# wheaton5/cellector

Measured on AMD Instinct MI355X. Metric: cell x locus log-likelihood evals/sec over full EM iterations (EM iters/sec in em_iters_per_s), higher is better.
Workload: dtype f64

## Files before the change

### cellector_amd/csrc/kernels_tiled.hip

```cpp
#include <hip/hip_ext.h>

#include "tiled.h"

__device__ __constant__ uint8_t T_A_OF[T_NCODE] = {1, 0, 2, 1, 0, 3, 2, 1, 0, 4, 3, 2, 1, 0};
__device__ __constant__ uint8_t T_R_OF[T_NCODE] = {0, 1, 0, 1, 2, 0, 1, 2, 3, 0, 1, 2, 3, 4};

struct ab_src_t {
    const double *s_alt, *s_ref, *alt_min, *ref_min;
    const uint8_t *mask;
    double2 *ab_out;
    double *xl_counters;
    uint32_t *d_counters, *tile_work;
    uint32_t n_work;
};
template <bool PAIRS>
__global__ __launch_bounds__(64 * TB_PARTS) void k_build_tables(uint64_t L, uint32_t nj, const double2 *__restrict__ ab,
                                                                const double *__restrict__ lf, double *__restrict__ tab,
                                                                ab_src_t src)
{
    if (src.s_alt && blockIdx.x == 0) {
        if (threadIdx.x < LC_COUNTERS) src.xl_counters[threadIdx.x] = 0.0;
        if (threadIdx.x < 8) src.d_counters[threadIdx.x] = 0u;
        for (uint32_t i = threadIdx.x; i < src.n_work; i += blockDim.x) src.tile_work[i] = 0u;
    }
    const int part = threadIdx.x >> 6;
    const uint64_t t = (uint64_t)blockIdx.x * 64 + (threadIdx.x & 63);
    if (t >= (uint64_t)nj * T_BL) return;
    const uint64_t chunk = t / T_BL, slot = t % T_BL;
    const uint64_t l = chunk * T_BLU + slot;
    double2 p = make_double2(-1.0, -1.0);
    if (slot < T_BLU && l < L) {
        if (src.s_alt) {
            p.x = (src.s_alt[l] + 1.0) - src.alt_min[l];
            p.y = (src.s_ref[l] + 1.0) - src.ref_min[l];
            if (!src.mask[l]) p.x = p.y = -1.0;
            if (part == 0) src.ab_out[l] = p;
        } else {
            p = ab[l];
        }
    }
    const bool live = p.x >= 0.0;
    double *img = tab + chunk * TAB_ELEMS;
#define TB_PMF(W, A, R) img[tab_pmf<geo_reg>((uint32_t)slot, W)] = live ? dm_log_bb_pmf(lf, p.x, p.y, A, R) : 0.0
#define TB_EXP(N) img[tab_exp<geo_reg>((uint32_t)slot, N - 1)] = (PAIRS && live) ? dm_expected_log_pmf(lf, p.x, p.y, N) : 0.0
    switch (part) {
    case 0: TB_EXP(4u); TB_PMF(0, 1u, 0u); break;
    case 1: TB_EXP(3u); TB_PMF(1, 0u, 1u); break;
    case 2: TB_EXP(2u); TB_PMF(2, 2u, 0u); TB_PMF(3, 1u, 1u); break;
    case 3: TB_EXP(1u); TB_PMF(4, 0u, 2u); TB_PMF(5, 3u, 0u); break;
    case 4: TB_PMF(6, 2u, 1u); TB_PMF(7, 1u, 2u); TB_PMF(8, 0u, 3u); TB_PMF(9, 4u, 0u); break;
    default: TB_PMF(10, 3u, 1u); TB_PMF(11, 2u, 2u); TB_PMF(12, 1u, 3u); TB_PMF(13, 0u, 4u); break;
    }
#undef TB_PMF
#undef TB_EXP
}

#ifndef TILE_ABL
#define TILE_ABL 0
#endif
#ifndef TILE_PFD
#define TILE_PFD 2
#endif
#ifndef TILE_PFD_T2
#define TILE_PFD_T2 2
#endif
#ifndef TILE_PINNED
#define TILE_PINNED 1
#endif
#if TILE_ABL == 7
#define TILE_BARRIER() do { } while (0)
#else
#define TILE_BARRIER() asm volatile("s_waitcnt lgkmcnt(0)\n\ts_barrier" ::: "memory")
#endif

struct __attribute__((packed, aligned(4))) tile_u4 { uint32_t x, y, z, w; };

template <bool EXPECTED, int T_SB, class G = geo_reg>
__global__ __launch_bounds__(T_THREADS, 4) void k_tile_ll(uint32_t nb, uint32_t nj, uint32_t cpg, uint32_t groups,
                                                          uint32_t n_cols, uint32_t *__restrict__ work ,
                                                          const uint16_t *__restrict__ thdr,
                                                          const uint16_t *__restrict__ tiles,
                                                          const double *__restrict__ tab, uint64_t npad,
                                                          double *__restrict__ part_ll, double *__restrict__ part_ell)
{
    using tab_t = typename std::conditional<EXPECTED, double2, double>::type;
    constexpr uint32_t TAB_U = G::LROW * G::BL * sizeof(double) / 16;
    constexpr int NP = (TAB_U + T_THREADS - 1) / T_THREADS;
    static_assert(NP == 6, "table prefetch registers are written out by hand");
    __shared__ __attribute__((aligned(16))) double s_tab[G::LROW * G::BL];
    static_assert(G::LROW * G::BL % 2 == 0, "whole 16-byte units");
    __shared__ tab_t s_acc[T_SB * T_BC];
    __shared__ uint32_t s_col;
    const uint32_t tid = threadIdx.x, wv = tid >> 6, lane = tid & 63;
    const uint32_t g = blockIdx.x % groups;
    const uint32_t j0 = g * cpg, j1 = min(nj, j0 + cpg);
    if (j0 >= j1) return;
  for (;;) {
    if (tid == 0) s_col = atomicAdd(&work[g], 1u);
    __syncthreads();
    const uint32_t col = s_col;
    if (col >= n_cols) break;
    const uint32_t b0 = col * T_SB;
#pragma unroll
    for (int s = 0; s < T_SB; s++) {
        if constexpr (EXPECTED) s_acc[s * T_BC + tid] = make_double2(0.0, 0.0);
        else s_acc[s * T_BC + tid] = 0.0;
    }

    double2 p_t0, p_t1, p_t2, p_t3, p_t4, p_t5;
#define TABLE_PREFETCH(J)                                                                                        \
    do {                                                                                                         \
        const double2 *src__ = reinterpret_cast<const double2 *>(tab) + (uint64_t)(J) * TAB_U + tid;             \
        p_t0 = src__[0];                                                                                         \
        p_t1 = src__[T_THREADS];                                                                                 \
        p_t2 = src__[2 * T_THREADS];                                                                             \
        p_t3 = src__[3 * T_THREADS];                                                                             \
        p_t4 = src__[4 * T_THREADS];                                                                             \
        p_t5 = src__[5 * T_THREADS];                      \
    } while (0)

    struct row_t { tile_u4 lo, hi; uint32_t k; uint64_t base; };
    const uint32_t wv_s = (uint32_t)__builtin_amdgcn_readfirstlane((int)wv);
#define HDR_LOAD(H, J, S)            \
    do {                                                                                                         \
         \
         \
         \
        const uint32_t rot__ = (wv_s + 8u * ((uint32_t)(S) >> 1)) & 15u, sl__ = ((S) & 1u) ? 15u - rot__ : rot__; \
        if (TILE_ABL != 9 || first_rows)  \
        (H) = reinterpret_cast<const uint4 *>(thdr + ((uint64_t)min(b0 + (uint32_t)(S), nb - 1) * nj + (TILE_ABL == 10 ? j0 : (J))) * T_HDR)[sl__]; \
    } while (0)
#define ROW_LOAD(E, H)                                                                                           \
    do {                                                                                                         \
        (E).k = (SKIP_EMPTY && (H).w) ? 0u : (H).z;  \
        (E).base = ((uint64_t)(H).y << 32) | (H).x;                                                              \
         \
         \
        const char *sb__ = reinterpret_cast<const char *>(tiles + (E).base);                                     \
        const uint32_t off__ = __umul24(lane, ((H).z + 1u) * 2u);                      \
        if ((!(TILE_ABL == 2 || TILE_ABL == 9) || first_rows) && !(SKIP_EMPTY && (H).w)) {  \
            (E).lo = *reinterpret_cast<const tile_u4 *>(sb__ + off__);                                           \
            (E).hi = *reinterpret_cast<const tile_u4 *>(sb__ + ((H).z > 7u ? 16u : 0u) + off__);                 \
        }                                                                                                        \
    } while (0)

    constexpr bool SKIP_EMPTY = G::NLO != 1;
    constexpr uint32_t PFD = T_SB == 4 ? (uint32_t)(G::NLO == 1 ? TILE_PFD : TILE_PFD_T2) : 2u;
    static_assert(PFD >= 2 && PFD <= 4, "row buffers");
    uint4 h0, h1, h2, h3;
    row_t e0, e1, e2, e3;
    bool first_rows = true;
    TABLE_PREFETCH(j0);
    __builtin_amdgcn_sched_barrier(0);
#define HDR_STEP(H, T) HDR_LOAD(H, min(j0 + (uint32_t)(T) / T_SB, j1 - 1), (uint32_t)(T) % T_SB)
    HDR_STEP(h0, 0);
    HDR_STEP(h1, 1);
    if constexpr (PFD >= 3) HDR_STEP(h2, 2);
    if constexpr (PFD == 4) HDR_STEP(h3, 3);
    ROW_LOAD(e0, h0);
    ROW_LOAD(e1, h1);
    if constexpr (PFD >= 3) ROW_LOAD(e2, h2);
    if constexpr (PFD == 4) ROW_LOAD(e3, h3);
    HDR_STEP(h0, PFD);
    HDR_STEP(h1, PFD + 1);
    if constexpr (PFD >= 3) HDR_STEP(h2, PFD + 2);
    if constexpr (PFD == 4) HDR_STEP(h3, PFD + 3);
#undef HDR_STEP
    first_rows = false;

#if TILE_ABL == 1 || TILE_ABL == 5
#define TILE_LOOKUP(V, E16) do { if constexpr (EXPECTED) V = make_double2((double)(E16), 1.0); else V = (double)(E16); } while (0)
#elif TILE_ABL == 4
#define TILE_LOOKUP(V, E16)                                                                                      \
    do {                                                                                                         \
        const uint32_t b__ = (((E16) >> 4) & 127u) * 32u + (lane & 31u), c__ = (((E16) >> 5) & 127u) * 32u + (lane & 31u); \
        if constexpr (EXPECTED) V = make_double2(s_tab[b__], s_tab[c__ + 4096u]);                                \
        else V = s_tab[b__];                                                                                     \
    } while (0)
#else
#define TILE_LOOKUP(V, E16)                                                                                      \
    do {                                                                                                         \
        const uint32_t s__ = ((E16) >> G::SHIFT) & G::SMASK;                                                     \
        if constexpr (EXPECTED) V = make_double2(s_tab[tab_pmf<G>(s__, (E16) & G::CMASK)], s_tab[tab_exp<G>(s__, (E16) >> 14)]); \
        else V = s_tab[tab_pmf<G>(s__, (E16) & G::CMASK)];                                                       \
    } while (0)
#endif
#define TILE_RD(V, KK)                                                                                           \
    tab_t V;                                                                                                     \
    do {                                                                                                         \
        const uint32_t idx__ = (((KK) + 1) & 1) ? (w__[((KK) + 1) >> 1] >> 16) : (w__[((KK) + 1) >> 1] & 0xffffu); \
        TILE_LOOKUP(V, idx__);                                                                                   \
    } while (0)
#define TILE_ADD(V)                                                                                              \
    do {                                                                                                         \
        if constexpr (EXPECTED) { a_ll__ += (V).x; a_el__ += (V).y; }                                            \
        else a_ll__ += (V);                                                                                      \
    } while (0)
#if TILE_PINNED
#define TILE_PIN(V)                                                                                              \
    do {                                                                                                         \
        if constexpr (EXPECTED) asm volatile("" : "+v"((V).x), "+v"((V).y) : : "memory");                        \
        else asm volatile("" : "+v"(V) : : "memory");                                                            \
    } while (0)
#else
#define TILE_PIN(V) do { } while (0)
#endif
#define TILE_LEVEL(KA, KB, PA, PB, BODY)                                                                         \
    if (K__ > (KA)) {                                                                                            \
        TILE_RD(v##KA, KA); TILE_RD(v##KB, KB);                                                                  \
        TILE_PIN(PA); TILE_PIN(PB);                                                                              \
        TILE_ADD(PA); TILE_ADD(PB);                                                                              \
        BODY                                                                                                     \
    } else { TILE_ADD(PA); TILE_ADD(PB); }
#define TILE_STEP(S, E, H)                                                                                       \
    do {                                                                                                         \
         \
        const uint32_t w__[8] = {(E).lo.x, (E).lo.y, (E).lo.z, (E).lo.w, (E).hi.x, (E).hi.y, (E).hi.z, (E).hi.w}; \
        const uint32_t K__ = (uint32_t)__builtin_amdgcn_readfirstlane((int)(E).k);        \
        const uint64_t cur_base__ = (E).base;                                                                    \
        const uint32_t cell__ = w__[0] & 0xffffu;                                                                \
              \
        ROW_LOAD(E, H);                                                                                          \
        HDR_LOAD(H, min(j + ((S) + 2 * PFD) / T_SB, j1 - 1), ((S) + 2 * PFD) % T_SB);                            \
         \
          \
        if (!(SKIP_EMPTY && K__ == 0u)) {                                                                        \
        tab_t acc__;                                                                                             \
        if constexpr (TILE_ABL == 8) { if constexpr (EXPECTED) acc__ = make_double2(0.0, 0.0); else acc__ = 0.0; }        \
        else acc__ = s_acc[(S) * T_BC + (TILE_ABL == 6 ? tid : cell__)];                                         \
        double a_ll__ = 0.0, a_el__ = 0.0;                                                                       \
          \
        TILE_RD(v0, 0);                                                                                          \
        if (K__ > 1) {                                                                                           \
            TILE_RD(v1, 1); TILE_RD(v2, 2);                                                                      \
            TILE_PIN(v0);                                                                                        \
            TILE_ADD(v0);                                                                                        \
            TILE_LEVEL(3, 4, v1, v2,                                                                             \
            TILE_LEVEL(5, 6, v3, v4,                                                                             \
            TILE_LEVEL(7, 8, v5, v6,                                                                             \
            TILE_LEVEL(9, 10, v7, v8,                                                                            \
            TILE_LEVEL(11, 12, v9, v10,                                                                          \
            TILE_LEVEL(13, 14, v11, v12,                                                                         \
                TILE_ADD(v13); TILE_ADD(v14);                                                                    \
                for (uint32_t k = T_NE; k < K__; k++) {  \
                    tab_t v__;                                                                                   \
                    TILE_LOOKUP(v__, (uint32_t)(tiles + cur_base__ + lane * (K__ + 1u))[k + 1]);                 \
                    TILE_ADD(v__);                                                                               \
                } ))))))                                                                                         \
        } else TILE_ADD(v0);                                                                                     \
         \
         \
        if constexpr (EXPECTED) { acc__.x += a_ll__; acc__.y += a_el__; }                                        \
        else acc__ += a_ll__;                                                                                    \
        if (TILE_ABL != 8 || a_ll__ == 12345.678) s_acc[(S) * T_BC + (TILE_ABL == 6 ? tid : cell__)] = acc__;   \
        }                                                                                                        \
    } while (0)

    static_assert(T_SB == 2 || T_SB == 4, "even and odd steps use different pipeline buffers");
#if TILE_ABL == 3 || TILE_ABL == 5 || TILE_ABL == 7
#define TILE_STAGE_IF if (j == j0)
#define TILE_NEXT_TABLE() do { } while (0)
#else
#define TILE_STAGE_IF
#define TILE_NEXT_TABLE() TABLE_PREFETCH(min(j + 1, j1 - 1))
#endif
#define TILE_STAGE()                                                                                             \
    do {                                                                                                         \
        TILE_BARRIER();  \
        TILE_STAGE_IF {                                                                                          \
            double2 *dst = reinterpret_cast<double2 *>(s_tab) + tid;                                             \
            dst[0] = p_t0;                                                                                       \
            dst[T_THREADS] = p_t1;                                                                               \
            dst[2 * T_THREADS] = p_t2;                                                                           \
            dst[3 * T_THREADS] = p_t3;                                                                           \
            dst[4 * T_THREADS] = p_t4;                                                                           \
            if (tid + 5 * T_THREADS < TAB_U) dst[5 * T_THREADS] = p_t5;                                          \
        }                                                                                                        \
        TILE_NEXT_TABLE();                                                                                       \
        TILE_BARRIER();                                                                       \
    } while (0)
    if constexpr (T_SB == 4 && PFD == 3) {
        for (uint32_t j = j0;;) {
            TILE_STAGE();
            TILE_STEP(0, e0, h0); TILE_STEP(1, e1, h1); TILE_STEP(2, e2, h2); TILE_STEP(3, e0, h0);
            if (++j >= j1) break;
            TILE_STAGE();
            TILE_STEP(0, e1, h1); TILE_STEP(1, e2, h2); TILE_STEP(2, e0, h0); TILE_STEP(3, e1, h1);
            if (++j >= j1) break;
            TILE_STAGE();
            TILE_STEP(0, e2, h2); TILE_STEP(1, e0, h0); TILE_STEP(2, e1, h1); TILE_STEP(3, e2, h2);
            if (++j >= j1) break;
        }
    } else {
        for (uint32_t j = j0; j < j1; j++) {
            TILE_STAGE();
            TILE_STEP(0, e0, h0);
            TILE_STEP(1, e1, h1);
            if constexpr (T_SB == 4 && PFD == 4) {
                TILE_STEP(2, e2, h2);
                TILE_STEP(3, e3, h3);
            } else if constexpr (T_SB == 4) {
                TILE_STEP(2, e0, h0);
                TILE_STEP(3, e1, h1);
            }
        }
    }
#undef TILE_STAGE
#undef TILE_STAGE_IF
#undef TILE_NEXT_TABLE
    TILE_BARRIER();
#pragma unroll
    for (int s = 0; s < T_SB; s++) {
        if (b0 + s < nb) {
            const uint64_t c = (uint64_t)g * npad + (uint64_t)(b0 + s) * T_BC + tid;
            const tab_t a = s_acc[s * T_BC + tid];
            if constexpr (EXPECTED) { part_ll[c] = a.x; part_ell[c] = a.y; }
            else part_ll[c] = a;
        }
    }
    __builtin_amdgcn_s_waitcnt(0);
  }
#undef TILE_STEP
#undef TILE_LEVEL
#undef TILE_PIN
#undef TILE_ADD
#undef TILE_RD
#undef TILE_LOOKUP
#undef ROW_LOAD
#undef HDR_LOAD
#undef TABLE_PREFETCH
}

template <typename T>
__device__ __forceinline__ T group16_sum(T v)
{
#pragma unroll
    for (int m = LF_LANES / 2; m > 0; m >>= 1) v += __shfl_xor(v, m, LF_LANES);
    return v;
}

__device__ __noinline__ double ov_slow_log_pmf(const double *lf, double alpha, double beta, uint32_t a, uint32_t r)
{
    return dm_log_bb_pmf(lf, alpha, beta, a, r);
}

__device__ __forceinline__ double ov_rcp(double y)
{
    const double r = __builtin_amdgcn_rcp(y);
    return __builtin_fma(__builtin_fma(-y, r, 1.0), r, r);
}
__device__ __forceinline__ double ov_expected_rec(double alpha, double beta, uint32_t n)
{
    const double ab = alpha + beta;
    double p = 1.0;
    for (uint32_t j = 0; j < n; ++j) p *= (beta + (double)j) * ov_rcp(ab + (double)j);
    double s = p * p;
    for (uint32_t k = 0; k < n; ++k) {
        p *= ((double)(n - k) * (alpha + (double)k)) * ov_rcp((double)(k + 1) * (beta + (double)(n - k - 1)));
        s += p * p;
    }
    return log(s);
}

__global__ __launch_bounds__(256) void k_ovf_tables(uint64_t L, const double2 *__restrict__ ab, const uint32_t *__restrict__ nmask,
                                                    double *__restrict__ otab)
{
    const uint64_t idx = (uint64_t)blockIdx.x * 256 + threadIdx.x;
    const uint64_t l = idx / 3;
    if (l >= L) return;
    const int fam = (int)(idx % 3);
    const double2 p = ab[l];
    double *row = otab + l * OV_ROW + fam * OV_NT;
    if (!(p.x >= 0.0)) {
        if (fam == 0) row[0] = -1.0;
        return;
    }
    const uint32_t m = nmask[l];
    const int top = m ? 4 + (31 - __clz((int)m)) : 0;
    const double x0 = fam == 0 ? p.x : (fam == 1 ? p.y : p.x + p.y);
    double acc = 0.0;
    row[0] = 0.0;
    for (int i = 0; i < OV_NT - 1 && i < top; i++) {
        acc += log(x0 + (double)i);
        row[i + 1] = acc;
    }
}
__global__ __launch_bounds__(256) void k_ovf_tables_e(uint64_t L, const double2 *__restrict__ ab,
                                                      const uint32_t *__restrict__ nmask, double *__restrict__ otab,
                                                      double *__restrict__ etab )
{
    const uint64_t idx = (uint64_t)blockIdx.x * 256 + threadIdx.x;
    const uint64_t l = idx >> 4;
    if (l >= L) return;
    const uint32_t i = (uint32_t)(idx & 15u);
    if (i == 15u) {
        if (etab) *reinterpret_cast<double2 *>(etab + l * OV_REC) = ab[l];
        return;
    }
    if (i > (uint32_t)OV_NE - 4u || !((nmask[l] >> i) & 1u)) return;
    const double2 p = ab[l];
    if (!(p.x >= 0.0)) return;
    const double e = ov_expected_rec(p.x, p.y, 4u + i);
    otab[l * OV_ROW + OV_EOFF + i] = e;
    if (etab && i >= 1 && i <= 4) etab[l * OV_REC + 2 + (i - 1)] = e;
}

__global__ __launch_bounds__(256) void k_ovf_values(uint64_t n_ovf, const uint32_t *__restrict__ ovc_locus,
                                                    const uint64_t *__restrict__ ovc_ent,
                                                    const double2 *__restrict__ ab, const double *__restrict__ lf,
                                                    const double *__restrict__ otab, double *__restrict__ lp_out)
{
    const uint64_t i = (uint64_t)blockIdx.x * 256 + threadIdx.x;
    if (i >= n_ovf) return;
    const uint32_t l = ovc_locus[i];
    const uint64_t en = ovc_ent[i];
    const double *row = otab + (uint64_t)l * OV_ROW;
    double lp = 0.0;
    if (row[0] >= 0.0) {
        const uint32_t a = ENT_ALT(en), r = ENT_REF(en), n = a + r;
        if (n == 0) lp = 0.0;
        else if (n < (uint32_t)OV_NT) lp = (lf[n] - lf[a] - lf[r]) + (row[a] + row[OV_NT + r] - row[2 * OV_NT + n]);
        else {
            const double2 p = ab[l];
            lp = ov_slow_log_pmf(lf, p.x, p.y, a, r);
        }
    }
    lp_out[i] = lp;
}

template <bool EXPECTED, bool PACKED, bool FULL>
__global__ __launch_bounds__(256) void k_ovf_cell_direct(
    uint64_t n_rows, const uint64_t *__restrict__ ell_ptr, const uint64_t *__restrict__ ell,
    const double2 *__restrict__ ab, const double *__restrict__ lf, const double *__restrict__ etab,
    const double *__restrict__ otab, double *__restrict__ o_ll, double *__restrict__ o_ell)
{
    static_assert(EXPECTED || !PACKED, "the record is built for the EM pass");
    static_assert(!(FULL && PACKED), "the full form runs unthrottled: it takes the unpacked tables");
    const uint64_t row = (uint64_t)blockIdx.x * blockDim.x + threadIdx.x;
    if (row >= n_rows) return;
    double s = 0.0, e = 0.0;
    const uint64_t grp = row >> 6, base = ell_ptr[grp] + (row & 63), end = ell_ptr[grp + 1];
#pragma unroll 1
    for (uint64_t i = base; i < end; i += 64) {
        const uint64_t en = ell[i];
        if (en == OVF_PAD) continue;
        const uint32_t l = ENT_IDX(en), a = ENT_ALT(en), r = ENT_REF(en), n = a + r;
        const double *rec = etab + (uint64_t)l * OV_REC;
        const double2 p = PACKED ? *reinterpret_cast<const double2 *>(rec) : ab[l];
        double ev = 0.0;
        if (PACKED) ev = n > (uint32_t)T_K && n <= (uint32_t)OV_FAST_N ? rec[n - 3] : 0.0;
        if (!(p.x >= 0.0) || n == 0 || n > (uint32_t)(FULL ? OV_NE : OV_FAST_N)) continue;
        if (FULL && n > (uint32_t)OV_FAST_N) {
            s += (lf[n] - lf[a] - lf[r]) + dm_log_beta_ratio(p.x, p.y, a, r);
            if (EXPECTED) e += otab[(uint64_t)l * OV_ROW + OV_EOFF + (n - 4)];
            continue;
        }
        const double abs_ = p.x + p.y;
        double num = 1.0, den = 1.0;
        for (uint32_t k = 0; k < n; ++k) {
            num *= (k < a) ? (p.x + (double)k) : (p.y + (double)(k - a));
            den *= abs_ + (double)k;
        }
        s += (lf[n] - lf[a] - lf[r]) + log(num / den);
        if (EXPECTED) {
            if (PACKED) e += ev;
            else e += n >= 5 ? rec[2 + (n - 5)] : otab[(uint64_t)l * OV_ROW + OV_EOFF + (n - 4)];
        }
    }
    o_ll[row] = s;
    if (EXPECTED) o_ell[row] = e;
}

template <bool EXPECTED>
__global__ __launch_bounds__(256) void k_ovf_cell_wide(uint64_t n_rows, const uint64_t *__restrict__ ovf_ptr,
                                                       const uint64_t *__restrict__ ovf_ent, const double2 *__restrict__ ab,
                                                       const double *__restrict__ lf, const double *__restrict__ etab,
                                                       const double *__restrict__ otab, double *__restrict__ o_ll,
                                                       double *__restrict__ o_ell)
{
    const uint32_t j = threadIdx.x % LF_LANES;
// ... 1224 lines not shown
```

### cellector_amd/csrc/kernels_tiled_build.hip

```cpp
#include "tiled.h"

__device__ __forceinline__ uint64_t row_lower_bound(const uint64_t *__restrict__ ent, uint64_t lo, uint64_t hi, uint32_t locus)
{
    while (lo < hi) {
        const uint64_t mid = (lo + hi) >> 1;
        if (ENT_IDX(ent[mid]) < locus) lo = mid + 1; else hi = mid;
    }
    return lo;
}

template <class G>
__device__ __forceinline__ bool geo_take(uint64_t e)
{
    const uint32_t n = ENT_ALT(e) + ENT_REF(e);
    return n - G::NLO <= G::NHI - G::NLO;
}
template <class G>
__device__ __forceinline__ uint16_t geo_encode(uint64_t e, uint32_t j)
{
    const uint32_t r = ENT_REF(e), n = ENT_ALT(e) + r;
    const uint32_t code = G::NLO == 1 ? ent_code(e) : t2_code(n, r);
    return (uint16_t)(((n - G::NLO) << 14) | ((ENT_IDX(e) - j * G::BLU) << G::SHIFT) | code);
}
template <bool FILL, class G = geo_reg>
__global__ __launch_bounds__(T_BC) void k_tile_build(uint64_t nloc, uint32_t nj, uint64_t tile0,
                                                     const uint64_t *__restrict__ csr_ptr,
                                                     const uint64_t *__restrict__ csr_ent,
                                                     uint64_t *__restrict__ tile_elems ,
                                                     uint16_t *__restrict__ tiles, uint16_t *__restrict__ thdr,
                                                     const uint32_t *__restrict__ toff )
{
    __shared__ uint32_t s_cnt[T_BC / 64][TB_BINS];
    __shared__ uint32_t s_base[TB_BINS];
    __shared__ uint32_t s_kmax[T_BC / 64];
    __shared__ uint32_t s_sbase[T_BC / 64 + 1];
    const uint64_t t = tile0 + blockIdx.x;
    const uint32_t b = (uint32_t)(t / nj), j = (uint32_t)(t % nj);
    const uint32_t cl = threadIdx.x, lane = cl & 63, wv = cl >> 6;
    const uint64_t row = (uint64_t)b * T_BC + cl;
    for (uint32_t i = cl; i < (T_BC / 64) * TB_BINS; i += T_BC) (&s_cnt[0][0])[i] = 0;
    if (cl < T_BC / 64) s_kmax[cl] = 0;
    uint64_t lo = 0, hi = 0;
    uint32_t len = 0;
    if (row < nloc) {
        const uint64_t beg = csr_ptr[row], end = csr_ptr[row + 1];
        if (toff) {
            lo = beg + toff[row * (nj + 1) + j];
            hi = beg + toff[row * (nj + 1) + j + 1];
        } else {
            lo = row_lower_bound(csr_ent, beg, end, j * G::BLU);
            hi = row_lower_bound(csr_ent, lo, end, (j + 1u) * G::BLU);
        }
        for (uint64_t i = lo; i < hi; i++) len += geo_take<G>(csr_ent[i]) ? 1u : 0u;
    }
    __syncthreads();
    const uint32_t bin = min(len, (uint32_t)TB_BINS - 1u);
    uint32_t within = 0;
    {
        unsigned long long todo = ~0ull;
        while (todo) {
            const int src = __ffsll((long long)todo) - 1;
            const uint32_t v = (uint32_t)__shfl((int)bin, src, 64);
            const unsigned long long m = __ballot(bin == v);
            if (bin == v) within = (uint32_t)__popcll(m & ((1ull << lane) - 1ull));
            if ((int)lane == src) s_cnt[wv][v] = (uint32_t)__popcll(m);
            todo &= ~m;
        }
    }
    __syncthreads();
    if (cl < TB_BINS) {
        uint32_t tot = 0;
        for (int w = 0; w < T_BC / 64; w++) tot += s_cnt[w][cl];
        uint32_t inc = tot;
#pragma unroll
        for (int off = 1; off < 64; off <<= 1) {
            const uint32_t o = __shfl_up(inc, off, 64);
            if ((int)cl >= off) inc += o;
        }
        s_base[cl] = inc - tot;
    }
    __syncthreads();
    uint32_t rank = s_base[bin] + within;
    for (uint32_t w = 0; w < wv; w++) rank += s_cnt[w][bin];
    const uint32_t dw = rank >> 6, dl = rank & 63;
    atomicMax(&s_kmax[dw], len);
    __syncthreads();
    if (cl == 0) {
        uint32_t acc = 0;
        for (int w = 0; w < T_BC / 64; w++) {
            s_sbase[w] = acc;
            acc += 64u * ((s_kmax[w] | 1u) + 1u);
        }
        s_sbase[T_BC / 64] = acc;
    }
    __syncthreads();
    if (!FILL) {
        if (cl == 0) tile_elems[t] = (uint64_t)s_sbase[T_BC / 64];
        return;
    }
    const uint64_t tbase = tile_elems[t];
    uint16_t *hp = thdr + t * T_HDR;
    if (cl < T_BC / 64) {
        uint32_t *hd = reinterpret_cast<uint32_t *>(hp) + 4 * cl;
        const uint64_t first = tbase + s_sbase[cl];
        hd[0] = (uint32_t)first;
        hd[1] = (uint32_t)(first >> 32);
        hd[2] = s_kmax[cl] | 1u;
        hd[3] = s_kmax[cl] == 0u;
    }
    const uint32_t K = s_kmax[dw] | 1u;
    uint16_t *dst = tiles + tbase + s_sbase[dw] + dl * (K + 1u);
    dst[0] = (uint16_t)cl;
    uint32_t k = 0;
    for (uint64_t i = lo; i < hi; i++) {
        const uint64_t e = csr_ent[i];
        if (geo_take<G>(e)) dst[1 + k++] = geo_encode<G>(e, j);
    }
    for (; k < K; k++) dst[1 + k] = (uint16_t)(G::BLU << G::SHIFT);
}

#define TBO_ROUNDS 4
__device__ __forceinline__ void tbo_banks(uint32_t e, uint32_t *a, uint32_t *b)
{
    const uint32_t slot = (e >> geo_reg::SHIFT) & geo_reg::SMASK;
    *a = tab_pmf<geo_reg>(slot, e & geo_reg::CMASK) & 31u;
    *b = tab_exp<geo_reg>(slot, e >> 14) & 31u;
}
__device__ uint32_t tile_lane_assign(uint16_t *slice , uint32_t Kw, uint32_t lane, uint32_t cnt, uint32_t *scr)
{
#define TLA_SYNC() asm volatile("s_waitcnt lgkmcnt(0)" ::: "memory")
    const uint32_t cls = (uint32_t)slice[lane * (Kw + 1u)] & 15u;
    const unsigned long long lt = (1ull << lane) - 1ull;
    uint32_t t = 0;
#pragma unroll
    for (uint32_t c = 0; c < 16u; c++) {
        const unsigned long long m = __ballot(cls == c);
        if (c < cls) t += (uint32_t)__popcll(m);
        else if (c == cls) t += (uint32_t)__popcll(m & lt);
    }
    const uint32_t g = t & 3u, pp = ((t >> 2) + ((g & 1u) ? 8u : 0u)) & 15u;
    const uint32_t l0 = pp < 4u ? pp : (pp < 8u ? pp + 8u : pp + 12u);
    const uint32_t l1 = pp < 8u ? pp + 4u : (pp < 12u ? pp + 8u : pp + 16u);
    const uint32_t dst = ((g & 1u) ? l1 : l0) + ((g & 2u) ? 32u : 0u);
    scr[dst] = lane;
    scr[64 + dst] = cnt;
    TLA_SYNC();
    const uint32_t src = scr[lane], cnt_new = scr[64 + lane];
    for (uint32_t k = 0; k <= Kw; k++) {
        const uint16_t v = slice[src * (Kw + 1u) + k];
        TLA_SYNC();
        slice[lane * (Kw + 1u) + k] = v;
        TLA_SYNC();
    }
    return cnt_new;
#undef TLA_SYNC
}

#define TBO_WIN 4
__device__ void tile_bank_order(uint16_t *row , uint32_t K, uint32_t cnt ,
                                uint32_t lane, uint32_t *scr )
{
    const uint32_t h = lane >> 5;
    uint32_t *ld_a = scr + h * 64, *ld_b = ld_a + 32, *win_a = scr + 128 + h * 64, *win_b = win_a + 32;
#define TBO_SYNC() asm volatile("s_waitcnt lgkmcnt(0)" ::: "memory")
    if (K <= 1u) return;
    for (uint32_t k = 0; k + 1u < K; k++) {
        if (__ballot(k + 1u < cnt) == 0ull) break;
        scr[lane] = 0u; scr[64 + lane] = 0u;
        uint32_t e[TBO_WIN], ca[TBO_WIN], cb[TBO_WIN];
#pragma unroll
        for (uint32_t u = 0; u < (uint32_t)TBO_WIN; u++) {
            e[u] = k + u < cnt ? (uint32_t)row[k + u] : 0xffffffffu;
            tbo_banks(e[u], &ca[u], &cb[u]);
        }
        bool open = k < cnt;
        TBO_SYNC();
        for (uint32_t rd = 0; rd < (uint32_t)TBO_ROUNDS; rd++) {
            if (__ballot(open) == 0ull) break;
            scr[128 + lane] = ~0u; scr[192 + lane] = ~0u;
            uint32_t cost[TBO_WIN];
#pragma unroll
            for (uint32_t u = 0; u < (uint32_t)TBO_WIN; u++) cost[u] = ld_a[ca[u]] + ld_b[cb[u]];
            uint32_t best = 0, bc = cost[0];
#pragma unroll
            for (uint32_t u = 1; u < (uint32_t)TBO_WIN; u++)
                if (e[u] != 0xffffffffu && cost[u] < bc) { bc = cost[u]; best = u; }
            uint32_t ba = ca[0], bb = cb[0];
#pragma unroll
            for (uint32_t u = 1; u < (uint32_t)TBO_WIN; u++)
                if (best == u) { ba = ca[u]; bb = cb[u]; }
            TBO_SYNC();
            if (open) {
                atomicMin(&win_a[ba], lane);
                atomicMin(&win_b[bb], lane);
            }
            TBO_SYNC();
            if (open && (rd == (uint32_t)TBO_ROUNDS - 1u || (win_a[ba] == lane && win_b[bb] == lane))) {
                if (best) {
                    uint32_t eb = e[0];
#pragma unroll
                    for (uint32_t u = 1; u < (uint32_t)TBO_WIN; u++)
                        if (best == u) eb = e[u];
                    row[k] = (uint16_t)eb;
                    row[k + best] = (uint16_t)e[0];
                }
                atomicAdd(&ld_a[ba], 1u);
                atomicAdd(&ld_b[bb], 1u);
                open = false;
            }
            TBO_SYNC();
        }
    }
#undef TBO_SYNC
}

__device__ __constant__ uint8_t T_NM1_OF[16] = {0, 0, 1, 1, 1, 2, 2, 2, 2, 3, 3, 3, 3, 3, 0, 0};
template <bool FILL, bool ORDER = false>
__global__ __launch_bounds__(T_BC, 8) void k_tile_build2(uint64_t nloc, uint32_t nb, uint32_t nj, const uint64_t *__restrict__ csr_ptr,
                                                      const uint16_t *__restrict__ c4r, const uint32_t *__restrict__ toff ,
                                                      uint64_t *__restrict__ tile_elems ,
                                                      uint16_t *__restrict__ tiles, uint16_t *__restrict__ thdr)
{
    static_assert(T_BLU < LR_LOCI, "a chunk's loci are told apart by their low 12 bits");
    __shared__ uint32_t s_cnt[T_BC / 64][TB_BINS];
    __shared__ uint32_t s_base[TB_BINS];
    __shared__ uint32_t s_kmax[T_BC / 64];
    __shared__ uint32_t s_sbase[T_BC / 64 + 1];
    __shared__ __attribute__((aligned(16))) uint16_t s_tile[FILL ? TB_STAGE : 8];
    __shared__ uint32_t s_scr[ORDER ? (T_BC / 64) * 256 : 1];
    __shared__ uint16_t s_rcnt[ORDER ? T_BC : 1];
    const uint32_t cl = threadIdx.x, lane = cl & 63, wv = cl >> 6;
    for (uint32_t b = blockIdx.x; b < nb; b += gridDim.x) {
        const uint64_t row = (uint64_t)b * T_BC + cl;
        const bool have = row < nloc;
        const uint64_t beg = have ? csr_ptr[row] : 0;
        const uint32_t *orow = toff + (have ? row : 0) * ((uint64_t)nj + 1);
        uint32_t o_lo = have ? orow[0] : 0u, o_hi = have ? orow[1] : 0u;
        for (uint32_t j = 0; j < nj; j++) {
            const uint64_t t = (uint64_t)b * nj + j;
            for (uint32_t i = cl; i < (T_BC / 64) * TB_BINS; i += T_BC) (&s_cnt[0][0])[i] = 0;
            if (cl < T_BC / 64) s_kmax[cl] = 0;
            const uint32_t o_next = have ? orow[min(j + 2u, nj)] : 0u;
            const uint64_t lo = beg + o_lo, hi = beg + o_hi;
            constexpr uint32_t TB_SEG = 16;
            uint32_t seg[TB_SEG];
            if (FILL) {
#pragma unroll
                for (uint32_t u = 0; u < TB_SEG; u++) seg[u] = lo + u < hi ? (uint32_t)c4r[lo + u] : 0xffffu;
            }
            const uint32_t len = o_hi - o_lo;
            __syncthreads();
            const uint32_t bin = min(len, (uint32_t)TB_BINS - 1u);
            uint32_t within = 0;
            {
                unsigned long long todo = ~0ull;
                while (todo) {
                    const int src = __ffsll((long long)todo) - 1;
                    const uint32_t v = (uint32_t)__shfl((int)bin, src, 64);
                    const unsigned long long m = __ballot(bin == v);
                    if (bin == v) within = (uint32_t)__popcll(m & ((1ull << lane) - 1ull));
                    if ((int)lane == src) s_cnt[wv][v] = (uint32_t)__popcll(m);
                    todo &= ~m;
                }
            }
            __syncthreads();
            if (cl < TB_BINS) {
                uint32_t tot = 0;
                for (int w = 0; w < T_BC / 64; w++) tot += s_cnt[w][cl];
                uint32_t inc = tot;
#pragma unroll
                for (int off = 1; off < 64; off <<= 1) {
                    const uint32_t o = __shfl_up(inc, off, 64);
                    if ((int)cl >= off) inc += o;
                }
                s_base[cl] = inc - tot;
            }
            __syncthreads();
            uint32_t rank = s_base[bin] + within;
            for (uint32_t w = 0; w < wv; w++) rank += s_cnt[w][bin];
            const uint32_t dw = rank >> 6, dl = rank & 63;
            atomicMax(&s_kmax[dw], len);
            __syncthreads();
            if (cl == 0) {
                uint32_t acc = 0;
                for (int w = 0; w < T_BC / 64; w++) {
                    s_sbase[w] = acc;
                    acc += 64u * ((s_kmax[w] | 1u) + 1u);
                }
                s_sbase[T_BC / 64] = acc;
            }
            __syncthreads();
            const uint32_t total = s_sbase[T_BC / 64];
            if (!FILL) {
                if (cl == 0) tile_elems[t] = (uint64_t)total;
            } else {
                const uint64_t tbase = tile_elems[t];
                if (cl < T_BC / 64) {
                    uint32_t *hd = reinterpret_cast<uint32_t *>(thdr + t * T_HDR) + 4 * cl;
                    const uint64_t first = tbase + s_sbase[cl];
                    hd[0] = (uint32_t)first;
                    hd[1] = (uint32_t)(first >> 32);
                    hd[2] = s_kmax[cl] | 1u;
                    hd[3] = s_kmax[cl] == 0u;
                }
                const uint32_t K = s_kmax[dw] | 1u;
                const bool staged = total <= (uint32_t)TB_STAGE;
                uint16_t *dst = (staged ? s_tile : tiles + tbase) + s_sbase[dw] + dl * (K + 1u);
                dst[0] = (uint16_t)cl;
                uint32_t k = 0;
                const uint32_t cbase = (j * (uint32_t)T_BLU) & (LR_LOCI - 1u);
#define TB_PUT(E)                                                                                                       \
                do {                                                                                                   \
                    const uint32_t e__ = (E), code__ = e__ >> 12;                                                      \
                    if (code__ < (uint32_t)T_NCODE)                                                                    \
                        dst[1 + k++] = (uint16_t)(((uint32_t)T_NM1_OF[code__] << 14) |                                 \
                                                  ((((e__ & (LR_LOCI - 1u)) - cbase) & (LR_LOCI - 1u)) << 4) | code__); \
                } while (0)
#pragma unroll
                for (uint32_t u = 0; u < TB_SEG; u++) TB_PUT(seg[u]);
                for (uint64_t i = lo + TB_SEG; i < hi; i++) TB_PUT((uint32_t)c4r[i]);
#undef TB_PUT
                if (ORDER) s_rcnt[rank] = (uint16_t)k;
                for (; k < K; k++) dst[1 + k] = T_NULL;
                if (staged) {
                    __syncthreads();
                    if (ORDER) {
                        const uint32_t Kw = s_kmax[wv] | 1u;
                        const uint32_t rc = tile_lane_assign(s_tile + s_sbase[wv], Kw, lane, s_rcnt[wv * 64 + lane], s_scr + wv * 256);
                        tile_bank_order(s_tile + s_sbase[wv] + lane * (Kw + 1u) + 1u, Kw, rc, lane, s_scr + wv * 256);
                        __syncthreads();
                    }
                    uint4 *out = reinterpret_cast<uint4 *>(tiles + tbase);
                    const uint4 *in = reinterpret_cast<const uint4 *>(s_tile);
                    for (uint32_t i = cl; i < total / 8u; i += T_BC) out[i] = in[i];
                }
            }
            __syncthreads();
            o_lo = o_hi;
            o_hi = o_next;
        }
    }
}

template <bool FILL, int REST = 0>
__global__ __launch_bounds__(256) void k_ovf_build(uint64_t n_rows, const uint64_t *__restrict__ ptr,
                                                   const uint64_t *__restrict__ ent, uint64_t *__restrict__ optr,
                                                   uint64_t *__restrict__ oent)
{
    const int lane = threadIdx.x & 63;
    const uint64_t wave0 = (uint64_t)blockIdx.x * 4 + (threadIdx.x >> 6), nwaves = (uint64_t)gridDim.x * 4;
    for (uint64_t row = wave0; row < n_rows; row += nwaves) {
        const uint64_t beg = ptr[row], end = ptr[row + 1];
        uint64_t base = FILL ? optr[row] : 0, cnt = 0;
        for (uint64_t i0 = beg; i0 < end; i0 += 64) {
            const uint64_t i = i0 + lane;
            const uint64_t e = i < end ? ent[i] : 0;
            const bool ov = i < end && !ent_regular(e) && !(REST && ENT_ALT(e) + ENT_REF(e) - T2_NMIN <= (uint32_t)REST - T2_NMIN);
            const unsigned long long m = __ballot(ov);
            if (FILL && ov) oent[base + __popcll(m & ((1ull << lane) - 1ull))] = e;
            base += __popcll(m);
            cnt += __popcll(m);
        }
        if (!FILL && lane == 0) optr[row] = cnt;
    }
}

template <bool FILL, int EB>
__global__ __launch_bounds__(256) void k_c4_build(uint64_t L, const uint64_t *__restrict__ csc_ptr,
                                                  const uint64_t *__restrict__ csc_ent, uint64_t *__restrict__ c4_ptr,
                                                  uint32_t *__restrict__ c4_ent, uint32_t *__restrict__ hist_all)
{
    const int lane = threadIdx.x & 63;
    const uint64_t wave0 = (uint64_t)blockIdx.x * 4 + (threadIdx.x >> 6), nwaves = (uint64_t)gridDim.x * 4;
    for (uint64_t l = wave0; l < L; l += nwaves) {
        const uint64_t beg = csc_ptr[l], end = csc_ptr[l + 1];
        uint64_t base = FILL ? c4_ptr[l] : 0, cnt = 0;
        uint32_t myhist = 0;
        for (uint64_t i0 = beg; i0 < end; i0 += 64) {
            const uint64_t i = i0 + lane;
            const uint64_t e = i < end ? csc_ent[i] : 0;
            const bool reg = i < end && ent_regular(e);
            const uint32_t code = reg ? ent_code(e) : 0xffu;
            const unsigned long long m = __ballot(reg);
            if (FILL) {
                if (reg) c4_write1<EB>(c4_ent, base + __popcll(m & ((1ull << lane) - 1ull)), ENT_IDX(e), code);
            } else {
#pragma unroll
                for (int k = 0; k < T_NCODE; k++) {
                    const unsigned long long mk = __ballot(code == (uint32_t)k);
                    if (lane == k) myhist += (uint32_t)__popcll(mk);
                }
            }
            base += __popcll(m);
            cnt += __popcll(m);
        }
        if (!FILL) {
            if (lane == 0) c4_ptr[l] = (cnt + 3) & ~3ull;
            if (lane < T_NCODE) hist_all[l * T_NCODE + lane] = myhist;
        } else if ((uint64_t)lane < ((4 - (cnt & 3)) & 3)) {
            c4_write1<EB>(c4_ent, c4_ptr[l] + cnt + lane, EB == 32 ? 0x0fffffffu : 0xfffffu, 15u);
        }
    }
}

__global__ __launch_bounds__(256) void k_cell_compact(uint64_t nnz, const uint64_t *__restrict__ csr_ent, uint16_t *__restrict__ c4r)
{
    static_assert(LR_LOCI == 4096, "12 bits of locus inside its range + 4 bits of code");
    const uint64_t i = (uint64_t)blockIdx.x * 256 + threadIdx.x;
    if (i >= nnz) return;
    const uint64_t e = csr_ent[i];
    c4r[i] = (uint16_t)((ENT_IDX(e) % LR_LOCI) | ((ent_regular(e) ? ent_code(e) : 15u) << 12));
}

__global__ __launch_bounds__(256) void k_range_offsets(uint64_t n_rows, uint32_t R, uint32_t width,
                                                       const uint64_t *__restrict__ csr_ptr,
                                                       const uint64_t *__restrict__ csr_ent, uint32_t *__restrict__ roff)
{
    const int lane = threadIdx.x & 63;
    const uint64_t wave0 = (uint64_t)blockIdx.x * 4 + (threadIdx.x >> 6), nwaves = (uint64_t)gridDim.x * 4;
    for (uint64_t row = wave0; row < n_rows; row += nwaves) {
        const uint64_t beg = csr_ptr[row], end = csr_ptr[row + 1];
        uint32_t *o = roff + row * (R + 1);
        for (uint64_t i0 = beg; i0 <= end; i0 += 64) {
            const uint64_t i = i0 + lane;
            if (i > end) continue;
            const int r_prev = i > beg ? (int)(ENT_IDX(csr_ent[i - 1]) / width) : -1;
            const int r_here = i < end ? (int)(ENT_IDX(csr_ent[i]) / width) : (int)R;
            for (int r = r_prev + 1; r <= r_here; r++) o[r] = (uint32_t)(i - beg);
        }
    }
}

__global__ __launch_bounds__(256) void k_max_pair_entries(uint64_t n_rows, const uint64_t *__restrict__ csr_ptr,
                                                          const uint64_t *__restrict__ csr_ent, uint32_t *__restrict__ out)
{
    const int lane = threadIdx.x & 63;
    const uint64_t wave0 = (uint64_t)blockIdx.x * 4 + (threadIdx.x >> 6), nwaves = (uint64_t)gridDim.x * 4;
    uint32_t best = 1;
    for (uint64_t row = wave0; row < n_rows; row += nwaves) {
        const uint64_t beg = csr_ptr[row], end = csr_ptr[row + 1];
        for (uint64_t i = beg + 1 + lane; i < end; i += 64) {
            const uint64_t l = ENT_IDX(csr_ent[i]);
            if (ENT_IDX(csr_ent[i - 1]) != l) continue;
            if (i - 1 > beg && ENT_IDX(csr_ent[i - 2]) == l) continue;
            uint32_t run = 2;
            for (uint64_t k = i + 1; k < end && ENT_IDX(csr_ent[k]) == l; k++) run++;
            best = max(best, run);
        }
    }
    if (best > 1) atomicMax(out, best);
}

__global__ __launch_bounds__(256) void k_ovf_locus_ids(uint64_t L, const uint64_t *__restrict__ ovc_ptr, uint32_t *__restrict__ ovc_locus)
{
    const int lane = threadIdx.x & 63;
    const uint64_t wave0 = (uint64_t)blockIdx.x * 4 + (threadIdx.x >> 6), nwaves = (uint64_t)gridDim.x * 4;
    for (uint64_t l = wave0; l < L; l += nwaves)
        for (uint64_t i = ovc_ptr[l] + lane; i < ovc_ptr[l + 1]; i += 64) ovc_locus[i] = (uint32_t)l;
}

__global__ __launch_bounds__(256) void k_ovf_nmask(uint64_t L, const uint64_t *__restrict__ ovc_ptr,
                                                   const uint64_t *__restrict__ ovc_ent, uint32_t *__restrict__ nmask)
{
    const int lane = threadIdx.x & 63;
    const uint64_t wave0 = (uint64_t)blockIdx.x * 4 + (threadIdx.x >> 6), nwaves = (uint64_t)gridDim.x * 4;
    for (uint64_t l = wave0; l < L; l += nwaves) {
        uint32_t m = 0;
        for (uint64_t i = ovc_ptr[l] + lane; i < ovc_ptr[l + 1]; i += 64) {
            const uint64_t en = ovc_ent[i];
            const uint32_t n = ENT_ALT(en) + ENT_REF(en);
            if (n >= 4u && n <= (uint32_t)OV_NE) m |= 1u << (n - 4u);
        }
#pragma unroll
        for (int off = 32; off > 0; off >>= 1) m |= (uint32_t)__shfl_xor((int)m, off, 64);
        if (lane == 0) nmask[l] = m;
    }
}

template <bool FILL>
__global__ __launch_bounds__(256) void k_t2_lists(uint64_t L, const uint32_t *__restrict__ hist_all2, uint64_t *__restrict__ np,
                                                  uint64_t *__restrict__ ns, uint32_t *__restrict__ plist, uint32_t *__restrict__ slist,
                                                  uint32_t *__restrict__ pmask )
// ... 360 lines not shown
```

### cellector_amd/csrc/tiled.h

```cpp
#pragma once
#include <algorithm>
#include <initializer_list>
#include <type_traits>

#include "ctx.h"
#include "device_math.h"

#define T_K 4
#define T_NCODE 14
#ifndef T_LROW
#define T_LROW 18
#endif
#ifndef T_BL
#define T_BL 640
#endif
#define T_BLU (T_BL - 1)
#define T_BC 1024
#define T_THREADS 1024
static_assert(T_BC == T_ROWS_PER_TILE, "cellector_engine_info derives the lookup count from this");
#define T_SB_MAX 4
#define T_GROUPS_MAX 64
static_assert(T_GROUPS_MAX == CELLECTOR_TILE_WORK_STRIDE, "k_alpha_beta resets the counters with this stride");
#define T_GROUPS 8
#define T_NE 15
#define T_NULL ((uint16_t)(T_BLU << 4))
#define T_HDR 128
#define TAB_ELEMS ((uint64_t)T_LROW * T_BL)

__device__ __forceinline__ bool ent_regular(uint64_t e)
{
    const uint32_t n = ENT_ALT(e) + ENT_REF(e);
    return n >= 1u && n <= (uint32_t)T_K;
}
__device__ __forceinline__ uint32_t ent_code(uint64_t e)
{
    const uint32_t r = ENT_REF(e), n = ENT_ALT(e) + r;
    return n * (n + 1u) / 2u - 1u + r;
}

#define TB_PARTS 6

#ifndef TILE_CM
#define TILE_CM 1
#endif
struct geo_reg {
    static constexpr uint32_t LROW = T_LROW, BL = T_BL, NCODE = T_NCODE, SHIFT = 4, SMASK = 1023u, CMASK = 15u;
    static constexpr uint32_t BLU = BL - 1, NLO = 1, NHI = T_K;
    static constexpr bool CODE_MAJOR = TILE_CM != 0;
};
template <int NMAX>
struct geo_t2 {
    static_assert(NMAX == 6 || NMAX == 8, "tier-2 tile geometries");
    static constexpr uint32_t NCODE = NMAX == 8 ? 30 : 13, NE = NMAX - 4, LROW = NCODE + NE;
    static constexpr uint32_t BL = NMAX == 8 ? 339 : 768, SHIFT = NMAX == 8 ? 5 : 4, SMASK = NMAX == 8 ? 511u : 1023u,
                              CMASK = NMAX == 8 ? 31u : 15u;
    static constexpr uint32_t BLU = BL - 1, NLO = 5, NHI = NMAX;
    static constexpr bool CODE_MAJOR = false;
};
template <class G>
__host__ __device__ __forceinline__ constexpr uint32_t tab_pmf(uint32_t slot, uint32_t code)
{
    return G::CODE_MAJOR ? (G::LROW - G::NCODE + code) * G::BL + slot : slot * G::LROW + code;
}
template <class G>
__host__ __device__ __forceinline__ constexpr uint32_t tab_exp(uint32_t slot, uint32_t ne)
{
    return G::CODE_MAJOR ? ne * G::BL + slot : slot * G::LROW + G::NCODE + ne;
}

#define LF_LANES 16
#define OV_NT 18
#define OV_NE 17
#define OV_FAST_N DM_CHUNK
#define OV_ROW 128
#define OV_EOFF 64
#define OV_REC 8
#define OVF_PAD (~0ull)

#define T2_NMIN 5u
#define T2_NMAX 8u
#define T2_NCODE 30
#define T2_CSTRIDE 32
#define T2_ROW 48
static_assert(T2_NMAX == (unsigned)OV_FAST_N, "the tier lists take the totals above tier 2");
__device__ __forceinline__ bool t2_total(uint32_t n) { return n - T2_NMIN <= T2_NMAX - T2_NMIN; }
__device__ __forceinline__ uint32_t t2_code(uint32_t n, uint32_t r) { return n * (n + 1u) / 2u - 15u + r; }
__device__ __forceinline__ uint32_t t2_pos(uint32_t n, uint32_t r)
{
    const uint32_t hi = r >= 7u ? 1u : 0u;
    return ((n - T2_NMIN) + (n == 8u ? 1u : 0u) + hi) * 8u + 1u + (hi ? r - 7u : r);
}
__device__ __forceinline__ int ovf_tier(uint64_t en)
{
    const uint32_t n = ENT_ALT(en) + ENT_REF(en);
    return n <= (uint32_t)OV_FAST_N ? -1 : (n <= (uint32_t)OV_NE ? 0 : 1);
}

template <int EB>
__device__ __forceinline__ void c4_read1(const uint32_t *__restrict__ base, uint64_t i, uint32_t *cell, uint32_t *code)
{
    if (EB == 32) {
        const uint32_t x = base[i];
        *cell = x & 0x0fffffffu;
        *code = x >> 28;
    } else {
        const uint8_t *b = reinterpret_cast<const uint8_t *>(base) + 3 * i;
        const uint32_t v = (uint32_t)b[0] | ((uint32_t)b[1] << 8) | ((uint32_t)b[2] << 16);
        *cell = v & 0xfffffu;
        *code = v >> 20;
    }
}
template <int EB>
__device__ __forceinline__ void c4_write1(uint32_t *__restrict__ base, uint64_t i, uint32_t cell, uint32_t code)
{
    if (EB == 32) {
        base[i] = cell | (code << 28);
    } else {
        uint8_t *b = reinterpret_cast<uint8_t *>(base) + 3 * i;
        const uint32_t v = cell | (code << 20);
        b[0] = (uint8_t)v; b[1] = (uint8_t)(v >> 8); b[2] = (uint8_t)(v >> 16);
    }
}
#define LM_NUM 1
#define LM_DEN 8

#define LR_LOCI 4096
#define LR_SUB_MAX 16
#define LR_THREADS 1024
#define LR_GROUP 64
#define LR_ROW (LR_LOCI + 2)
#define LT_CELLS 64
#define TB_BINS 64
#define TB_STAGE (24 * 1024)

static inline unsigned gcap(uint64_t n, unsigned per_block, unsigned cap = 1u << 20)
{
    uint64_t g = (n + per_block - 1) / per_block;
    if (g < 1) g = 1;
    if (g > cap) g = cap;
    return (unsigned)g;
}

template <class F>
static inline void with_bool(bool b, F &&f)
{
    if (b) f(std::true_type());
    else f(std::false_type());
}

struct CountedPtr { uint64_t *ptr, *total; };
template <class Pass, class Payload>
static inline cellector_status count_scan_fill(cellector_ctx *c, uint64_t n, std::initializer_list<CountedPtr> a, Pass pass,
                                               Payload payload)
{
    pass(std::false_type());
    HIPCHK(c, hipGetLastError());
    for (const CountedPtr &p : a) CHK(dev_exclusive_scan_u64(c, p.ptr, n + 1, p.total));
    CHK(payload());
    pass(std::true_type());
    HIPCHK(c, hipGetLastError());
    return CELLECTOR_OK;
}
```

Before: 1083 billion.

## Store even-length tile rows without padding, moving cell ids to a slice header

Tile slices used to round every row length up to odd so each row (cell id plus entries) was a whole number of 32-bit words, which padded even-length rows with null entries. Now even-length rows are stored unpadded, with the 64 cell ids in a separate header block ahead of the rows. Odd rows keep the inline-cell layout. The evaluate kernel gets the cell id with a separate 16-bit load and handles the first entry explicitly for even rows, so fewer null lookups are done and less tile memory is read, at the cost of an extra load and more branching.

```diff
diff --git a/cellector_amd/csrc/kernels_tiled.hip b/cellector_amd/csrc/kernels_tiled.hip
--- a/cellector_amd/csrc/kernels_tiled.hip
+++ b/cellector_amd/csrc/kernels_tiled.hip
@@ -119,7 +119,7 @@
         p_t5 = src__[5 * T_THREADS];                      \
     } while (0)
 
-    struct row_t { tile_u4 lo, hi; uint32_t k; uint64_t base; };
+    struct row_t { tile_u4 lo, hi; uint32_t cell, k; uint64_t base; };
     const uint32_t wv_s = (uint32_t)__builtin_amdgcn_readfirstlane((int)wv);
 #define HDR_LOAD(H, J, S)            \
     do {                                                                                                         \
@@ -137,13 +137,24 @@
          \
          \
         const char *sb__ = reinterpret_cast<const char *>(tiles + (E).base);                                     \
-        const uint32_t off__ = __umul24(lane, ((H).z + 1u) * 2u);                      \
+        const uint32_t odd__ = (H).z & 1u, n16__ = (H).z + odd__;                                 \
+        const uint32_t off__ = __umul24(lane, n16__ * 2u) + (odd__ ? 0u : 128u);  \
         if ((!(TILE_ABL == 2 || TILE_ABL == 9) || first_rows) && !(SKIP_EMPTY && (H).w)) {  \
+            if constexpr (SKIP_EMPTY) {  \
+                if (!odd__) (E).cell = *reinterpret_cast<const uint16_t *>(sb__ + lane * 2u);                    \
+            }                                                                                                    \
             (E).lo = *reinterpret_cast<const tile_u4 *>(sb__ + off__);                                           \
-            (E).hi = *reinterpret_cast<const tile_u4 *>(sb__ + ((H).z > 7u ? 16u : 0u) + off__);                 \
+            (E).hi = *reinterpret_cast<const tile_u4 *>(sb__ + (n16__ > 8u ? 16u : 0u) + off__);                 \
         }                                                                                                        \
     } while (0)
 
+#define CELL_LOAD(E)                                                                                             \
+    do {                                                                                                         \
+        const uint32_t k__ = (E).k, odd__ = k__ & 1u;                                                            \
+        if constexpr (!SKIP_EMPTY)                                                                               \
+        (E).cell = *reinterpret_cast<const uint16_t *>(reinterpret_cast<const char *>(tiles + (E).base) +        \
+                                                       __umul24(lane, odd__ ? (k__ + 1u) * 2u : 2u));            \
+    } while (0)
     constexpr bool SKIP_EMPTY = G::NLO != 1;
     constexpr uint32_t PFD = T_SB == 4 ? (uint32_t)(G::NLO == 1 ? TILE_PFD : TILE_PFD_T2) : 2u;
     static_assert(PFD >= 2 && PFD <= 4, "row buffers");
@@ -161,6 +172,10 @@
     ROW_LOAD(e1, h1);
     if constexpr (PFD >= 3) ROW_LOAD(e2, h2);
     if constexpr (PFD == 4) ROW_LOAD(e3, h3);
+    CELL_LOAD(e0);
+    CELL_LOAD(e1);
+    if constexpr (PFD >= 3) CELL_LOAD(e2);
+    if constexpr (PFD == 4) CELL_LOAD(e3);
     HDR_STEP(h0, PFD);
     HDR_STEP(h1, PFD + 1);
     if constexpr (PFD >= 3) HDR_STEP(h2, PFD + 2);
@@ -206,7 +221,7 @@
 #define TILE_PIN(V) do { } while (0)
 #endif
 #define TILE_LEVEL(KA, KB, PA, PB, BODY)                                                                         \
-    if (K__ > (KA)) {                                                                                            \
+    if (D__ > (((KA) + 1u) >> 1)) {                                                                              \
         TILE_RD(v##KA, KA); TILE_RD(v##KB, KB);                                                                  \
         TILE_PIN(PA); TILE_PIN(PB);                                                                              \
         TILE_ADD(PA); TILE_ADD(PB);                                                                              \
@@ -216,10 +231,12 @@
     do {                                                                                                         \
          \
         const uint32_t w__[8] = {(E).lo.x, (E).lo.y, (E).lo.z, (E).lo.w, (E).hi.x, (E).hi.y, (E).hi.z, (E).hi.w}; \
-        const uint32_t K__ = (uint32_t)__builtin_amdgcn_readfirstlane((int)(E).k);        \
+        const uint32_t K__ = (uint32_t)__builtin_amdgcn_readfirstlane((int)(E).k);             \
+        const uint32_t D__ = (K__ + 1u) >> 1;                           \
         const uint64_t cur_base__ = (E).base;                                                                    \
-        const uint32_t cell__ = w__[0] & 0xffffu;                                                                \
-              \
+        const uint32_t cell__ = (SKIP_EMPTY && (K__ & 1u)) ? (w__[0] & 0xffffu) : (E).cell;                      \
+         \
+                                                                                  \
         ROW_LOAD(E, H);                                                                                          \
         HDR_LOAD(H, min(j + ((S) + 2 * PFD) / T_SB, j1 - 1), ((S) + 2 * PFD) % T_SB);                            \
          \
@@ -229,9 +246,15 @@
         if constexpr (TILE_ABL == 8) { if constexpr (EXPECTED) acc__ = make_double2(0.0, 0.0); else acc__ = 0.0; }        \
         else acc__ = s_acc[(S) * T_BC + (TILE_ABL == 6 ? tid : cell__)];                                         \
         double a_ll__ = 0.0, a_el__ = 0.0;                                                                       \
+        if (!(K__ & 1u)) {  \
+            tab_t vz__;                                                                                          \
+            TILE_LOOKUP(vz__, w__[0] & 0xffffu);                                                                 \
+            if constexpr (EXPECTED) { a_ll__ = vz__.x; a_el__ = vz__.y; }                                        \
+            else a_ll__ = vz__;                                                                                  \
+        }                                                                                                        \
           \
         TILE_RD(v0, 0);                                                                                          \
-        if (K__ > 1) {                                                                                           \
+        if (D__ > 1u) {                                                                                          \
             TILE_RD(v1, 1); TILE_RD(v2, 2);                                                                      \
             TILE_PIN(v0);                                                                                        \
             TILE_ADD(v0);                                                                                        \
@@ -242,9 +265,14 @@
             TILE_LEVEL(11, 12, v9, v10,                                                                          \
             TILE_LEVEL(13, 14, v11, v12,                                                                         \
                 TILE_ADD(v13); TILE_ADD(v14);                                                                    \
-                for (uint32_t k = T_NE; k < K__; k++) {  \
+                const uint32_t n16__ = K__ + (K__ & 1u);                                        \
+                for (uint32_t i = T_ROW_U16; i < n16__; i++) {  \
                     tab_t v__;                                                                                   \
-                    TILE_LOOKUP(v__, (uint32_t)(tiles + cur_base__ + lane * (K__ + 1u))[k + 1]);                 \
+                    uint32_t x__ = (tiles + cur_base__ + ((K__ & 1u) ? 0u : 64u) + lane * n16__)[i];             \
+                     \
+                                                               \
+                    asm volatile("" : "+v"(x__));                                                                \
+                    TILE_LOOKUP(v__, x__);                                                                       \
                     TILE_ADD(v__);                                                                               \
                 } ))))))                                                                                         \
         } else TILE_ADD(v0);                                                                                     \
@@ -254,6 +282,7 @@
         else acc__ += a_ll__;                                                                                    \
         if (TILE_ABL != 8 || a_ll__ == 12345.678) s_acc[(S) * T_BC + (TILE_ABL == 6 ? tid : cell__)] = acc__;   \
         }                                                                                                        \
+        CELL_LOAD(E);                                                                                            \
     } while (0)
 
     static_assert(T_SB == 2 || T_SB == 4, "even and odd steps use different pipeline buffers");
@@ -326,6 +355,7 @@
 #undef TILE_ADD
 #undef TILE_RD
 #undef TILE_LOOKUP
+#undef CELL_LOAD
 #undef ROW_LOAD
 #undef HDR_LOAD
 #undef TABLE_PREFETCH
diff --git a/cellector_amd/csrc/kernels_tiled_build.hip b/cellector_amd/csrc/kernels_tiled_build.hip
--- a/cellector_amd/csrc/kernels_tiled_build.hip
+++ b/cellector_amd/csrc/kernels_tiled_build.hip
@@ -89,7 +89,7 @@
         uint32_t acc = 0;
         for (int w = 0; w < T_BC / 64; w++) {
             s_sbase[w] = acc;
-            acc += 64u * ((s_kmax[w] | 1u) + 1u);
+            acc += 64u * (slice_k(s_kmax[w]) + 1u);
         }
         s_sbase[T_BC / 64] = acc;
     }
@@ -105,18 +105,18 @@
         const uint64_t first = tbase + s_sbase[cl];
         hd[0] = (uint32_t)first;
         hd[1] = (uint32_t)(first >> 32);
-        hd[2] = s_kmax[cl] | 1u;
+        hd[2] = slice_k(s_kmax[cl]);
         hd[3] = s_kmax[cl] == 0u;
     }
-    const uint32_t K = s_kmax[dw] | 1u;
-    uint16_t *dst = tiles + tbase + s_sbase[dw] + dl * (K + 1u);
-    dst[0] = (uint16_t)cl;
+    const uint32_t K = slice_k(s_kmax[dw]);
+    uint16_t *sl = tiles + tbase + s_sbase[dw], *dst = sl + slice_row_at(K, dl);
+    sl[slice_cell_at(K, dl)] = (uint16_t)cl;
     uint32_t k = 0;
     for (uint64_t i = lo; i < hi; i++) {
         const uint64_t e = csr_ent[i];
-        if (geo_take<G>(e)) dst[1 + k++] = geo_encode<G>(e, j);
-    }
-    for (; k < K; k++) dst[1 + k] = (uint16_t)(G::BLU << G::SHIFT);
+        if (geo_take<G>(e)) dst[k++] = geo_encode<G>(e, j);
+    }
+    for (; k < K; k++) dst[k] = (uint16_t)(G::BLU << G::SHIFT);
 }
 
 #define TBO_ROUNDS 4
@@ -129,7 +129,7 @@
 __device__ uint32_t tile_lane_assign(uint16_t *slice , uint32_t Kw, uint32_t lane, uint32_t cnt, uint32_t *scr)
 {
 #define TLA_SYNC() asm volatile("s_waitcnt lgkmcnt(0)" ::: "memory")
-    const uint32_t cls = (uint32_t)slice[lane * (Kw + 1u)] & 15u;
+    const uint32_t cls = (uint32_t)slice[slice_cell_at(Kw, lane)] & 15u;
     const unsigned long long lt = (1ull << lane) - 1ull;
     uint32_t t = 0;
 #pragma unroll
@@ -147,9 +147,9 @@
     TLA_SYNC();
     const uint32_t src = scr[lane], cnt_new = scr[64 + lane];
     for (uint32_t k = 0; k <= Kw; k++) {
-        const uint16_t v = slice[src * (Kw + 1u) + k];
+        const uint16_t v = slice[k ? slice_row_at(Kw, src) + k - 1u : slice_cell_at(Kw, src)];
         TLA_SYNC();
-        slice[lane * (Kw + 1u) + k] = v;
+        slice[k ? slice_row_at(Kw, lane) + k - 1u : slice_cell_at(Kw, lane)] = v;
         TLA_SYNC();
     }
     return cnt_new;
@@ -285,7 +285,7 @@
                 uint32_t acc = 0;
                 for (int w = 0; w < T_BC / 64; w++) {
                     s_sbase[w] = acc;
-                    acc += 64u * ((s_kmax[w] | 1u) + 1u);
+                    acc += 64u * (slice_k(s_kmax[w]) + 1u);
                 }
                 s_sbase[T_BC / 64] = acc;
             }
@@ -300,20 +300,20 @@
                     const uint64_t first = tbase + s_sbase[cl];
                     hd[0] = (uint32_t)first;
                     hd[1] = (uint32_t)(first >> 32);
-                    hd[2] = s_kmax[cl] | 1u;
+                    hd[2] = slice_k(s_kmax[cl]);
                     hd[3] = s_kmax[cl] == 0u;
                 }
-                const uint32_t K = s_kmax[dw] | 1u;
+                const uint32_t K = slice_k(s_kmax[dw]);
                 const bool staged = total <= (uint32_t)TB_STAGE;
-                uint16_t *dst = (staged ? s_tile : tiles + tbase) + s_sbase[dw] + dl * (K + 1u);
-                dst[0] = (uint16_t)cl;
+                uint16_t *sl = (staged ? s_tile : tiles + tbase) + s_sbase[dw], *dst = sl + slice_row_at(K, dl);
+                sl[slice_cell_at(K, dl)] = (uint16_t)cl;
                 uint32_t k = 0;
                 const uint32_t cbase = (j * (uint32_t)T_BLU) & (LR_LOCI - 1u);
 #define TB_PUT(E)                                                                                                       \
                 do {                                                                                                   \
                     const uint32_t e__ = (E), code__ = e__ >> 12;                                                      \
                     if (code__ < (uint32_t)T_NCODE)                                                                    \
-                        dst[1 + k++] = (uint16_t)(((uint32_t)T_NM1_OF[code__] << 14) |                                 \
+                        dst[k++] = (uint16_t)(((uint32_t)T_NM1_OF[code__] << 14) |                                     \
                                                   ((((e__ & (LR_LOCI - 1u)) - cbase) & (LR_LOCI - 1u)) << 4) | code__); \
                 } while (0)
 #pragma unroll
@@ -321,13 +321,13 @@
                 for (uint64_t i = lo + TB_SEG; i < hi; i++) TB_PUT((uint32_t)c4r[i]);
 #undef TB_PUT
                 if (ORDER) s_rcnt[rank] = (uint16_t)k;
-                for (; k < K; k++) dst[1 + k] = T_NULL;
+                for (; k < K; k++) dst[k] = T_NULL;
                 if (staged) {
                     __syncthreads();
                     if (ORDER) {
-                        const uint32_t Kw = s_kmax[wv] | 1u;
+                        const uint32_t Kw = slice_k(s_kmax[wv]);
                         const uint32_t rc = tile_lane_assign(s_tile + s_sbase[wv], Kw, lane, s_rcnt[wv * 64 + lane], s_scr + wv * 256);
-                        tile_bank_order(s_tile + s_sbase[wv] + lane * (Kw + 1u) + 1u, Kw, rc, lane, s_scr + wv * 256);
+                        tile_bank_order(s_tile + s_sbase[wv] + slice_row_at(Kw, lane), Kw, rc, lane, s_scr + wv * 256);
                         __syncthreads();
                     }
                     uint4 *out = reinterpret_cast<uint4 *>(tiles + tbase);
diff --git a/cellector_amd/csrc/tiled.h b/cellector_amd/csrc/tiled.h
--- a/cellector_amd/csrc/tiled.h
+++ b/cellector_amd/csrc/tiled.h
@@ -22,9 +22,12 @@
 #define T_GROUPS_MAX 64
 static_assert(T_GROUPS_MAX == CELLECTOR_TILE_WORK_STRIDE, "k_alpha_beta resets the counters with this stride");
 #define T_GROUPS 8
-#define T_NE 15
+#define T_ROW_U16 16
 #define T_NULL ((uint16_t)(T_BLU << 4))
 #define T_HDR 128
+__host__ __device__ __forceinline__ constexpr uint32_t slice_cell_at(uint32_t K, uint32_t r) { return (K & 1u) ? r * (K + 1u) : r; }
+__host__ __device__ __forceinline__ constexpr uint32_t slice_row_at(uint32_t K, uint32_t r) { return (K & 1u) ? r * (K + 1u) + 1u : 64u + r * K; }
+__host__ __device__ __forceinline__ constexpr uint32_t slice_k(uint32_t longest) { return longest ? longest : 1u; }
 #define TAB_ELEMS ((uint64_t)T_LROW * T_BL)
 
 __device__ __forceinline__ bool ent_regular(uint64_t e)
```

New measurement: 1100 billion (median of 6 runs). +1.6%, better.
